# 959AI994/Multi-Gate-VAE

Measured on AMD Instinct MI355X. Metric: circuit-graphs/sec (train step), AIG-64k batch=64 per GPU, higher is better.
Workload: dtype f32 storage; dense products as bf16x3 split-precision MFMA, fp32 accumulate; 1 GPU; cfg2: DG_AE --type aig, 64 x 65536-node synthetic levelised DAGs per GPU (N=4194304, E=6558720, 120 levels), H=64, 4+4 rounds, layernorm, weights [1,4,4], negatives sampled; step includes the 7-scalar metrics copy (pinned, read one step behind); global_batch=64, parallelism=dp1

## Files before the change

include/mgvae_hip.h:

```cpp
#ifndef MGVAE_HIP_H
#define MGVAE_HIP_H
#include <stdint.h>
#ifdef __cplusplus
extern "C" {
#endif

#ifndef MGV_OK
#define MGV_OK 0
#define MGV_EINVAL (-1)
#define MGV_EUNSUPPORTED (-2)
#endif

int mgv_abi_version(void);

int mgv_struct_stage_fwd(int H, int64_t N, const float* h_in, const int32_t* nbr_ptr, const int32_t* nbr_idx,
                         const uint8_t* xcls, const float* xtab, int C, const float* Wc, const float* bc,
                         const float* Whh, const float* bhh, const float* ln_w, const float* ln_b, float ln_eps,
                         float* h_out, void* stream);
int mgv_struct_stage_bwd(int H, int64_t N, const float* h_in, const int32_t* nbr_ptr, const int32_t* nbr_idx,
                         const uint8_t* xcls, const float* xtab, int C, const float* Wc, const float* WcT,
                         const float* bc, const float* Whh, const float* WhhT, const float* bhh,
                         const float* ln_w, const float* ln_b, float ln_eps, const float* gy_direct,
                         const float* gy_agg, float* g_direct_out, float* g_agg_out, float* dWc, float* dbc,
                         float* dWhh, float* dbhh, float* dxtab, float* dln_w, float* dln_b, void* stream);
// ... 264 lines not shown
                      int32_t* scratch, int64_t scratch_ints, void* stream);
int mgv_colour_rep_rows(int64_t C, const int32_t* rep, const int32_t* nbr_ptr, const int32_t* prev, const uint8_t* xcls, int heavy_row,
                        int32_t* rptr, int32_t* own, uint8_t* xrep, int32_t* n_heavy, int32_t* scratch, int64_t scratch_ints, void* stream);
int mgv_colour_rep_lists(int64_t C, const int32_t* rep, const int32_t* nbr_ptr, const int32_t* nbr_idx, const int32_t* prev, const int32_t* rptr,
                         int32_t* ent, int32_t* row, void* stream);
int mgv_sorted_key_counts(int64_t n, const int32_t* sorted_keys, int64_t K, int32_t* counts, void* stream);
int mgv_seg_level_work_ints(int64_t G);
int mgv_seg_level_scan(int64_t G, const int32_t* counts, int seg, int32_t* work, int64_t work_ints, void* stream);
int mgv_seg_level_fill(int64_t G, int64_t n_seg, const int32_t* gid, int seg, int base, const int32_t* work, int32_t* seg_ptr, int32_t* out_row,
                       int32_t* gid_next, int32_t* counts_next, void* stream);

int mgv_digcn_scales(int64_t N, const int32_t* list_ptr, const int32_t* opp_ptr, float alpha, float beta, int self_loops,
                     float* r, float* c, void* stream);
int mgv_digcn_gather(int H, int64_t N, const float* y, const int32_t* nbr_ptr, const int32_t* nbr_idx, const float* outer,
                     const float* inner, const float* mask, int self_loops, int relu, int heavy_n, const int32_t* heavy_nodes,
                     float* out, void* stream);
int mgv_digcn_class_fwd(int H, int64_t N, const uint8_t* xcls, const float* T, int C, const int32_t* nbr_ptr, const int32_t* nbr_idx,
                        const float* outer, const float* inner, int self_loops, int relu, float* out, void* stream);
int mgv_digcn_class_bwd_ws_floats(int H, int64_t N);
int mgv_digcn_class_bwd(int H, int64_t N, const uint8_t* xcls, int C, const int32_t* nbr_ptr, const int32_t* nbr_idx, const float* outer,
                        const float* inner, int self_loops, const float* z, const float* dz, float* dT, float* workspace,
                        int64_t workspace_floats, void* stream);

#ifdef __cplusplus
}
#endif
#endif
```

multi-gate-vae_amd/csrc/linear_x3.hip:

```cpp
#include "mgv_x3.h"
#include "mgv_slab.h"
#include "../../include/mgvae_hip.h"

namespace mgv {

struct LinX3Args {
    int64_t N;
    const float* X1; int K1; int ld1;
    const float* X2; int K2; int ld2;
    const __bf16* wpack;
    const float* b;
    float* Y; int ldy;
    const float* R; int ldr;
    float* Y2; int ldy2;
    const float* dY; int lddy;
    float* dW; float* db;
    float* slab;
    const int32_t* order; const int32_t* tile_start; const int32_t* tile_count; const int32_t* tile_slot; const int32_t* tile_list;
    int64_t g_ntiles; int64_t g_wstride;
};

template <int M>
struct LinSplit {
    static_assert(M % 16 == 0, "column tiles of 16");
// ... 301 lines not shown
        if (tid < G::F4G) s_part[tid] = dbs;
        __syncthreads();
        constexpr int QPR = M / 4;
        if (tid < M) {
            const int c4 = tid / 4, e = tid % 4;
            float sum = 0.f;
            for (int t = c4; t < G::F4G && t < G::NT; t += QPR) { const float4 v = s_part[t]; sum += e == 0 ? v.x : e == 1 ? v.y : e == 2 ? v.z : v.w; }
            slab[M * K + tid] = sum;
        }
    }
}

template <int M, int K, int NW, int WI, bool GROUPED = false>
__global__ __launch_bounds__(64 * NW) void k_linear_wgrad_x3(LinX3Args a) {
    linear_wgrad_x3_body<M, K, NW, WI, GROUPED, false, 0>(a);
}

template <int M, int K, int NW, int WI, int KSR>
__global__ __launch_bounds__(64 * NW) __attribute__((amdgpu_waves_per_eu(4))) void k_linear_bwd_x3(LinX3Args a) {
    linear_wgrad_x3_body<M, K, NW, WI, false, true, KSR>(a);
}

__global__ __launch_bounds__(256) void k_wpack_bf16x3(const float* W, int R, int K, int ldw, int transpose, __bf16* hi, __bf16* lo) {
    const int total = R * K, ksn = K / 32;
    for (int o = blockIdx.x * 256 + threadIdx.x; o < total; o += gridDim.x * 256) {
        const int blk = o >> 9, within = o & 511, lane = within >> 3, e = within & 7;
        const int rt = blk / ksn, ks = blk % ksn;
        const int row = rt * 16 + (lane & 15), k = ks * 32 + (lane >> 4) * 8 + e;
        const float v = transpose ? W[(int64_t)k * ldw + row] : W[(int64_t)row * ldw + k];
        __bf16 h, l;
        split_bf16(v, h, l);
        hi[o] = h; lo[o] = l;
    }
}

template <int M, int K, bool GROUPED = false>
int launch_linear_fwd_x3(const LinX3Args& a, hipStream_t st) {
    using G = LinFwdGeom<M, K>;
    static bool set = false;
    if (!set) { hipFuncSetAttribute(reinterpret_cast<const void*>(k_linear_fwd_x3<M, K, GROUPED>), hipFuncAttributeMaxDynamicSharedMemorySize, 160 * 1024); set = true; }
    const int64_t ntiles = a.order ? a.g_ntiles : (a.N + kTileRows - 1) / kTileRows;
    int per_cu = 160 * 1024 / G::smem_bytes;
    per_cu = per_cu > 4 ? 4 : per_cu;
    hipLaunchKernelGGL((k_linear_fwd_x3<M, K, GROUPED>), dim3(grid_for(ntiles, per_cu)), dim3(kThreads), G::smem_bytes, st, a);
    MGV_LAUNCH_RET();
}

template <int M, int K, int NW, int WI, bool GROUPED = false>
int launch_linear_wgrad_x3(const LinX3Args& a, int64_t ws_floats, hipStream_t st) {
    using G = LinWgGeom<M, K, NW, WI>;
    static bool set = false;
    if (!set) { hipFuncSetAttribute(reinterpret_cast<const void*>(k_linear_wgrad_x3<M, K, NW, WI, GROUPED>), hipFuncAttributeMaxDynamicSharedMemorySize, 160 * 1024); set = true; }
    const int64_t ntiles = a.order ? a.g_ntiles : (a.N + kTileRows - 1) / kTileRows;
    int per_cu = 160 * 1024 / G::smem_bytes;
    const int cap = 1024 / G::NT;
    per_cu = per_cu > cap ? cap : per_cu;
// ... 149 lines not shown
```

multi-gate-vae_amd/csrc/mgv_x3.h:

```cpp
#pragma once
#include "mgv_common.h"

typedef __bf16 bf16x8 __attribute__((ext_vector_type(8)));
typedef __bf16 bf16x4 __attribute__((ext_vector_type(4)));

namespace mgv {

__device__ __forceinline__ void split_bf16(float x, __bf16& hi, __bf16& lo) {
    hi = (__bf16)x;
    lo = (__bf16)(x - (float)hi);
}

__device__ __forceinline__ void split4(const float4& v, bf16x4& hi, bf16x4& lo) {
    __bf16 h0, h1, h2, h3, l0, l1, l2, l3;
    split_bf16(v.x, h0, l0); split_bf16(v.y, h1, l1); split_bf16(v.z, h2, l2); split_bf16(v.w, h3, l3);
    hi = bf16x4{h0, h1, h2, h3};
    lo = bf16x4{l0, l1, l2, l3};
}

__device__ __forceinline__ bf16x8 ldfrag(const __bf16* p) { return *reinterpret_cast<const bf16x8*>(p); }
__device__ __forceinline__ bf16x8 ldfrag_global(const __bf16* p) {
    return *(const __attribute__((address_space(1))) bf16x8*)p;
}
__device__ __forceinline__ void st_bf4(__bf16* p, const bf16x4& v) { *reinterpret_cast<bf16x4*>(p) = v; }

__device__ __forceinline__ f32x4 mfma_bf16(const bf16x8& a, const bf16x8& b, f32x4 c) {
    return __builtin_amdgcn_mfma_f32_16x16x32_bf16(a, b, c, 0, 0, 0);
}

__device__ __forceinline__ void mma_x3(f32x4& c, const bf16x8& ahi, const bf16x8& alo, const bf16x8& bhi, const bf16x8& blo) {
    c = mfma_bf16(alo, bhi, c);
    c = mfma_bf16(ahi, blo, c);
    c = mfma_bf16(ahi, bhi, c);
}

typedef __bf16 bf16x4v __attribute__((ext_vector_type(4)));
__device__ __forceinline__ bf16x8 ldfrag_tr(const __bf16* plane, int ld, int k0, int c0) {
    const int lane = threadIdx.x & 63, q = lane >> 4, i16 = lane & 15;
    const __bf16* p = plane + (k0 + 8 * q + (i16 >> 2)) * ld + c0 + 4 * (i16 & 3);
    const bf16x4v lo = __builtin_amdgcn_ds_read_tr16_b64_v4bf16((__attribute__((address_space(3))) bf16x4v*)p);
// ... 20 lines not shown
```

multi-gate-vae_amd/deepgate/_hip.py:

```python
import ctypes
import os
import re

import torch

_HERE = os.path.dirname(os.path.abspath(__file__))
_PKG_ROOT = os.path.dirname(_HERE)
_REPO_ROOT = os.path.dirname(_PKG_ROOT)
LIB_PATH = os.environ.get('MGV_LIB', os.path.join(_PKG_ROOT, 'csrc', 'libmgvae_hip.so'))
HEADER_PATH = os.path.join(_REPO_ROOT, 'include', 'mgvae_hip.h')

_CTYPE = (('int64_t', ctypes.c_int64), ('uint64_t', ctypes.c_uint64), ('int32_t', ctypes.c_int32),
          ('float', ctypes.c_float), ('double', ctypes.c_double), ('int', ctypes.c_int))


class HipLibraryError(RuntimeError):
    pass


def parse_header(path=HEADER_PATH):
    with open(path) as f:
        text = f.read()
    text = re.sub(r'/\*.*?\*/', '', text, flags=re.S)
    text = re.sub(r'//[^\n]*', '', text)
# ... 19 lines not shown

_lib = None
_sigs = None


def load():
    global _lib, _sigs
    if _lib is not None:
        return _lib
    if not os.path.exists(LIB_PATH):
        raise HipLibraryError('%s not found: build it with `make -C %s` (or __graft_entry__.build()); '
                              'there is no CPU fallback for the DG_AE hot path' % (LIB_PATH, os.path.dirname(LIB_PATH)))
    lib = ctypes.CDLL(LIB_PATH)
    sigs = parse_header()
    for name, types in sigs.items():
        try:
            fn = getattr(lib, name)
        except AttributeError:
            raise HipLibraryError('%s is declared in %s but not exported by %s' % (name, HEADER_PATH, LIB_PATH))
        fn.argtypes = types
        fn.restype = ctypes.c_int
    _lib, _sigs = lib, sigs
    return lib


class _TensorPtr(ctypes.c_void_p):
    _keep = None


def ptr(t):
    if t is None:
        return None
    p = _TensorPtr(t.data_ptr())
    p._keep = t
    return p


_raw_stream = getattr(torch._C, '_cuda_getCurrentRawStream', None)


def stream():
    if _raw_stream is not None:
        return ctypes.c_void_p(_raw_stream(torch.cuda.current_device()))
    return ctypes.c_void_p(torch.cuda.current_stream().cuda_stream)


# ... 52 lines not shown
```

multi-gate-vae_amd/deepgate/_model_base.py:

```python
import os

import torch
from torch import nn

from . import ops
from .arch.mlp import MLP
from .arch.tfmlp import TFMlpAggr
from .data import plan_of
from .digae_layer import DirectedInnerProductDecoder
from .sampling import NegativeEdges, negative_sampling, negative_sampling_device

EPS = 1e-15
DEVICE_SAMPLER = True
MAX_LOGSTD = 10


class FunctionalModel(nn.Module):
    ENCODER_ATTR = 'struct_encoder'
    GATES = ()

    def __init__(self, struct_encoder, num_rounds=1, dim_hidden=128, enable_encode=True, enable_reverse=True):
        super().__init__()
        setattr(self, self.ENCODER_ATTR, struct_encoder)
        self.decoder = DirectedInnerProductDecoder()
        self.hs_linear = nn.Linear(dim_hidden * 2, dim_hidden)
        self.hs_decompose = nn.Linear(dim_hidden, dim_hidden * 2)
        self.num_rounds = num_rounds
        self.enable_encode = enable_encode
        self.enable_reverse = enable_reverse
        self.dim_hidden = dim_hidden
        self.dim_mlp = 32
        for name, _ in self.GATES:
            setattr(self, 'aggr_%s_func' % name, TFMlpAggr(dim_hidden * 2, dim_hidden))
        for name, _ in self.GATES:
            setattr(self, 'update_%s_func' % name, nn.GRU(dim_hidden, dim_hidden))
        self.readout_prob = MLP(dim_hidden, self.dim_mlp, 1, num_layer=3, p_drop=0.2, norm_layer='batchnorm',
                                act_layer='relu')
        self.last_confusion = None
        self.last_link_metrics = None

    def _sweep_params(self):
        parts = [getattr(self, 'aggr_%s_func' % n).composed(getattr(self, 'update_%s_func' % n)) for n, _ in self.GATES]
        return [torch.stack([p[i] for p in parts]) for i in range(5)]

    def forward(self, G, after_hs=None):
        if self.num_rounds < 1:
            raise ValueError('num_rounds must be >= 1')
        plan = plan_of(G, [gid for _, gid in self.GATES])
        dev = self.hs_linear.weight.device
        rows = torch.eye(6, dtype=torch.float32, device=dev)
        enc = getattr(self, self.ENCODER_ATTR)
        s, t = enc(None, None, G.edge_index, plan=plan, classes=(rows, plan.xcls))
        hs = ops.linear(s, self.hs_linear.weight, self.hs_linear.bias, x2=t)
        self._hs_ready = torch.cuda.Event()
        self._hs_ready.record()
        self._hs_pass = None
        self.after_hs_out = after_hs(hs) if after_hs is not None else None
        hs_in = self._hs_pass if self._hs_pass is not None else hs
        self._hs_pass = None
        hf = ops.FuncSweepFn.apply(plan, hs_in, *self._sweep_params())
        for _ in range(self.num_rounds - 1):
            au, Wvc, bvc, bih, _ = self._sweep_params()
            hf = ops.FuncSweepFn.apply(plan, hs_in, au, Wvc, bvc, bih, None, hf, self._round_gh(plan, hf))
        return hs, hf
# ... 131 lines not shown
```

multi-gate-vae_amd/deepgate/digae_layer.py:

```python
import torch
import torch.nn as nn

from . import ops
from .arch.gcn_conv import AggConv
from .graph_plan import GraphPlan

MAX_FEATURE_CLASSES = 8


def feature_classes(x):
    rows, inv = torch.unique(x, dim=0, return_inverse=True)
    if rows.shape[0] > MAX_FEATURE_CLASSES:
        return None
    return rows.to(torch.float32), inv.to(torch.uint8).contiguous()


class DirectedInnerProductDecoder(nn.Module):

    def forward(self, s, t, edge_index, sigmoid=True):
        return ops.edge_dot(s, t, edge_index, sigmoid)

    def forward_all(self, s, t, sigmoid=True):
        return ops.pair_scores(s, t, sigmoid)

# ... 147 lines not shown
        for aggr, gru in ((self.aggr, self.update), (self.aggr_r, self.update_r)):
            w_ih = gru.weight_ih_l0
            w_m = w_ih[:, :H]
            w_x = torch.nn.functional.pad(w_ih[:, H:], (0, pad))
            xrow = torch.cat([ops.linear(xp, w_x[g * H:(g + 1) * H], gru.bias_ih_l0[g * H:(g + 1) * H]) for g in range(3)], dim=1)
            args += [xrow, w_m @ aggr.msg.weight, w_m @ aggr.msg.bias, gru.weight_hh_l0, gru.bias_hh_l0]
        ln_w = self.ln.weight if self.layernorm else None
        ln_b = self.ln.bias if self.layernorm else None
        return ops.StructEncoderRowsFn.apply(plan, self.num_rounds, *args, ln_w, ln_b)

    def forward(self, x, edge_index, plan=None, classes=None):
        if classes is None:
            if x.shape[1] != self.dim_feature:
                raise ValueError('expected %d node features, got %d' % (self.dim_feature, x.shape[1]))
            classes = feature_classes(x)
        if classes is None:
            return self._forward_rows(x, edge_index, plan)
        rows, xcls = classes
        if rows.shape[1] != self.dim_feature:
            raise ValueError('expected %d node features, got %d' % (self.dim_feature, rows.shape[1]))
        if plan is None:
            plan = GraphPlan(edge_index, xcls.shape[0])
        rows = rows.to(self.update.weight_ih_l0.device)
        f = self._composed(self.aggr, self.update, rows)
        r = self._composed(self.aggr_r, self.update_r, rows)
        ln_w = self.ln.weight if self.layernorm else None
        ln_b = self.ln.bias if self.layernorm else None
        return ops.StructEncoderFn.apply(plan, xcls, self.num_rounds, *f, *r, ln_w, ln_b)


class DirectMultiGCNEncoder(nn.Module):
    def __init__(self, dim_feature=3, dim_hidden=128, s_rounds=1, t_rounds=1, enable_reverse=True, layernorm=False):
        super().__init__()
        self.source_conv = MultiGCNEncoder(s_rounds, dim_hidden, dim_feature, enable_reverse, layernorm)
        self.target_conv = MultiGCNEncoder(t_rounds, dim_hidden, dim_feature, enable_reverse, layernorm)

    def forward(self, s, t, edge_index, plan=None, classes=None):
        if plan is None:
            plan = GraphPlan(edge_index, s.shape[0])
        cs = classes if classes is not None else feature_classes(s)
        ct = cs if (classes is not None or t is s) else feature_classes(t)
        return self.source_conv(s, edge_index, plan, cs), self.target_conv(t, edge_index, plan, ct)
```

multi-gate-vae_amd/deepgate/ops.py:

```python
from collections import namedtuple

import torch

from . import _hip
from ._hip import HipLibraryError, check, ptr

import os

F32 = torch.float32
I32 = torch.int32
U8 = torch.uint8
LN_EPS = 1e-5

PRECISION = os.environ.get('MGV_PRECISION', 'x3')
FIRST_STAGE_TABLE = True


def use_x3(H):
    return PRECISION == 'x3' and H in (32, 64)


def split_bf16(w):
    hi = w.to(torch.bfloat16)
    lo = (w - hi.to(torch.float32)).to(torch.bfloat16)
    return hi, lo


def frag_order(w):
    R, K = w.shape
    return w.reshape(R // 16, 16, K // 32, 4, 8).permute(0, 2, 3, 1, 4).reshape(-1)


def _pack_into(out, off, W, transpose):
    R, K = (W.shape[1], W.shape[0]) if transpose else W.shape
    n = W.numel()
    if W.dtype != F32 or not W.is_cuda or W.stride(1) != 1:
        raise HipLibraryError('weight must be an fp32 GPU matrix with contiguous rows')
    base = out.data_ptr() + 2 * off
    _hip.call('mgv_wpack_bf16x3', ptr(W), R, K, W.stride(0), int(transpose), _hip.ctypes.c_void_p(base),
              _hip.ctypes.c_void_p(base + 2 * n))
    return off + 2 * n


def stage_wpack(Wc, Whh):
    out = torch.empty(4 * (Wc.numel() + Whh.numel()), dtype=torch.bfloat16, device=Wc.device)
    off = 0
    for w, tr in ((Wc, False), (Whh, False), (Wc, True), (Whh, True)):
        off = _pack_into(out, off, w, tr)
    return out


def sweep_wpack(Wvc):
    out = torch.empty(4 * Wvc.numel(), dtype=torch.bfloat16, device=Wvc.device)
    off = 0
    for g in range(Wvc.shape[0]):
        off = _pack_into(out, off, Wvc[g], False)
        off = _pack_into(out, off, Wvc[g], True)
    return out


def linear_wpack(W):
    out = torch.empty(2 * W.numel(), dtype=torch.bfloat16, device=W.device)
    _pack_into(out, 0, W, False)
    return out


def _zeros_like_params(*ts):
    return [torch.zeros_like(t) for t in ts]


def _heavy_args(heavy, H, device):
    if heavy is None or heavy[0] == 0:
        return 0, None, None
    n, nodes = heavy
    return n, ptr(nodes), ptr(workspace(2 * n * H, device, tag='heavy'))


def struct_stage_fwd(h_in, nbr_ptr, nbr_idx, xcls, xtab, Wc, bc, Whh, bhh, ln_w, ln_b, out=None, wpack=None, heavy=None, table_own=None, n_rows=None,
                     stats_out=None, tagged=True):
    N, H = h_in.shape
    if n_rows is not None:
        N = int(n_rows)
    if table_own is not None:
        N = table_own.numel()
    check(h_in, F32, 'h_in'); check(nbr_ptr, I32, 'nbr_ptr'); check(nbr_idx, I32, 'nbr_idx'); check(xcls, U8, 'xcls')
    for n, t in (('xtab', xtab), ('Wc', Wc), ('bc', bc), ('Whh', Whh), ('bhh', bhh)):
        check(t, F32, n)
    check(ln_w, F32, 'ln_w'); check(ln_b, F32, 'ln_b')
    assert nbr_ptr.numel() == N + 1 and xcls.numel() == N
    assert Wc.shape == (3 * H, H) and Whh.shape == (3 * H, H) and xtab.shape[1] == 3 * H
    h_out = (torch.empty(N, H, dtype=F32, device=h_in.device) if out is None else out)
# ... 97 lines not shown
                     dict(idx=st['idx'], n_rows=st['C'], src='stacked', own=st['own']))
            out.append(HalfRound(rev, st['C'], st['ptr'], xcls=st['xcls'], heavy=st['heavy'], expand=st['cid'] if k + 1 == q else None,
                                 grad=grad, gsrc=gsrc, **lists))
        elif k == 0 and first is not None:
            cid, C, tp, ti, tx = first
            out.append(HalfRound(rev, C, tp, ti, tx, None, src='ones', expand=None if table_mode else cid, grad='pairs', gsrc=(cid, p, i)))
        elif k == 1 and table_mode:
            out.append(HalfRound(rev, N, p, plan.tagged_idx(rev, first[0]), xcls, plan.heavy(rev), table_own=first[0]))
        else:
            out.append(HalfRound(rev, N, p, i, xcls, plan.heavy(rev), src='ones' if k == 0 else 'prev'))
    return out


class StructEncoderFn(torch.autograd.Function):

    @staticmethod
    def forward(ctx, plan, xcls, rounds, xtab_f, Wc_f, bc_f, Whh_f, bhh_f, xtab_r, Wc_r, bc_r, Whh_r, bhh_r, ln_w, ln_b):
        N = plan.N
        H = Whh_f.shape[1]
        dev = Whh_f.device
        par = [t.detach().contiguous() for t in (xtab_f, Wc_f, bc_f, Whh_f, bhh_f, xtab_r, Wc_r, bc_r, Whh_r, bhh_r)]
        lw = ln_w.detach().contiguous() if ln_w is not None else None
        lb = ln_b.detach().contiguous() if ln_b is not None else None
        packs = (stage_wpack(par[1], par[3]), stage_wpack(par[6], par[8])) if use_x3(H) else (None, None)
        quot = plan.quotient(xcls, 2 * rounds) if (QUOTIENT and FIRST_STAGE_TABLE and rounds > 0 and N > 0 and Whh_f.is_cuda) else []
        first = plan.first_stage_classes(xcls) if (not quot and FIRST_STAGE_TABLE and rounds > 0 and N > 0) else None
        sched = half_round_schedule(plan, xcls, rounds, H, use_x3(H), first, quot)
        keep_stats = lw is not None and use_x3(H) and H == 64
        states, stats = [], []
        h = torch.ones(1, H, dtype=F32, device=dev) if quot else None
        for r in sched:
            if r.src == 'ones':
                h = torch.ones(r.rows, H, dtype=F32, device=dev)
            elif r.src == 'stacked':
                h = torch.cat([h.index_select(0, r.own), h])
            states.append(None if r.grad == 'pairs' else h)
            stats.append(torch.empty(r.rows, 2, dtype=F32, device=dev) if keep_stats else None)
            h = struct_stage_fwd(h, r.ptr, r.idx, r.xcls, *(par[5:] if r.rev else par[:5]), lw, lb, wpack=packs[int(r.rev)], heavy=r.heavy,
                                 table_own=r.table_own, n_rows=r.n_rows, stats_out=stats[-1], tagged=r.tagged)
            if r.expand is not None:
                table, h = h, torch.empty(N, H, dtype=F32, device=dev)
                _hip.call('mgv_class_expand', H, N, ptr(table), ptr(r.expand), ptr(h))
        if not sched:
            h = torch.ones(N, H, dtype=F32, device=dev)
        ctx.plan, ctx.packs, ctx.sched = plan, packs, sched
        ctx.par, ctx.lw, ctx.lb, ctx.states, ctx.stats = par, lw, lb, states, stats
        return h

    @staticmethod
    def backward(ctx, gy):
        plan, par, lw, lb = ctx.plan, ctx.par, ctx.lw, ctx.lb
        H, dev = gy.shape[1], gy.device
        dlw = torch.zeros_like(lw) if lw is not None else None
        dlb = torch.zeros_like(lb) if lb is not None else None
        acc = [dict(zip(('dxtab', 'dWc', 'dbc', 'dWhh', 'dbhh', 'dln_w', 'dln_b'), _zeros_like_params(*w) + [dlw, dlb])) for w in (par[:5], par[5:])]
        g_direct, g_agg = gy.contiguous(), None
        for k in range(len(ctx.sched) - 1, -1, -1):
            r, h_in = ctx.sched[k], ctx.states[k]
            if r.grad == 'pairs':
                cid, p, i = r.gsrc
                gsum = torch.zeros(r.rows, H, dtype=F32, device=dev)
                ws = workspace(_hip.call_value('mgv_class_pull_sum_ws_floats', H, plan.N, r.rows), dev)
                _hip.call('mgv_class_pull_sum', H, plan.N, ptr(g_direct), ptr(g_agg), ptr(p), ptr(i), ptr(cid), r.rows, ptr(gsum), ptr(ws), ws.numel())
                g_direct, g_agg, h_in = gsum, None, torch.ones(r.rows, H, dtype=F32, device=dev)
            elif r.grad == 'sum_levels':
                (order, levels), p, i = r.gsrc
                g_direct, g_agg = _seg_sums(H, levels, order, g_direct, g_agg, p, i), None
            elif r.grad == 'above':
                own_levels, own_rows, ent_levels, ent_rows = r.gsrc
                g_direct, g_agg = _seg_sums(H, own_levels, own_rows, g_direct) + _seg_sums(H, ent_levels, ent_rows, g_agg), None
            g_direct, g_agg = struct_stage_bwd(h_in, r.ptr, r.idx, r.xcls, *(par[5:] if r.rev else par[:5]), lw, lb, g_direct, g_agg, acc[int(r.rev)],
                                               need_input_grad=(k > 0), wpack=ctx.packs[int(r.rev)], heavy=r.heavy, table_own=r.table_own,
                                               n_rows=r.n_rows, stats=ctx.stats[k], tagged=r.tagged)
        ctx.states = ctx.stats = None
        f, r = acc
        return (None, None, None, f['dxtab'], f['dWc'], f['dbc'], f['dWhh'], f['dbhh'],
                r['dxtab'], r['dWc'], r['dbc'], r['dWhh'], r['dbhh'], dlw, dlb)

# ... 28 lines not shown
        acc = {}
        for tag, w in (('f', par[:5]), ('r', par[5:])):
            acc[tag] = [torch.zeros_like(t) for t in w]
            acc[tag] += [w[1].t().contiguous(), w[3].t().contiguous()]
        dlw = torch.zeros_like(lw) if lw is not None else None
        dlb = torch.zeros_like(lb) if lb is not None else None
        g_direct, g_agg = gy.contiguous(), None
        k = len(ctx.states) - 1
        for _ in range(ctx.rounds):
            for rev in (True, False):
                p, i = plan.csr(rev)
                w = par[5:] if rev else par[:5]
                g = acc['r' if rev else 'f']
                gd = torch.empty(N, H, dtype=F32, device=dev) if k > 0 else None
                ga = torch.empty(N, H, dtype=F32, device=dev) if k > 0 else None
                _hip.call('mgv_struct_stage_rows_bwd', H, N, ptr(ctx.states[k]), ptr(p), ptr(i), ptr(w[0]), ptr(w[1]), ptr(g[5]), ptr(w[2]),
                          ptr(w[3]), ptr(g[6]), ptr(w[4]), ptr(lw), ptr(lb), LN_EPS, ptr(g_direct), ptr(g_agg), ptr(gd), ptr(ga),
                          ptr(g[1]), ptr(g[2]), ptr(g[3]), ptr(g[4]), ptr(g[0]), ptr(dlw), ptr(dlb))
                g_direct, g_agg = gd, ga
                k -= 1
        ctx.states = None
        f, r = acc['f'], acc['r']
        return (None, None, f[0], f[1], f[2], f[3], f[4], r[0], r[1], r[2], r[3], r[4], dlw, dlb)


_LIN_X3 = {}


def _lin_x3(M, K):
    if PRECISION != 'x3':
        return False
    key = (int(M), int(K))
    if key not in _LIN_X3:
        _LIN_X3[key] = bool(_hip.call_value('mgv_linear_x3_supported', *key))
    return _LIN_X3[key]


FUSED_LINEAR_BWD = os.environ.get('MGV_FUSED_LINEAR_BWD', '1') != '0'


def _lin_bwd_x3(M, K):
    if PRECISION != 'x3':
        return False
    key = ('bwd', int(M), int(K))
    if key not in _LIN_X3:
        _LIN_X3[key] = bool(_hip.call_value('mgv_linear_bwd_x3_supported', int(M), int(K)))
# ... 359 lines not shown
            _hip.call('mgv_func_sweep_fwd', H, N, T, plan.num_levels, ltp, ptr(plan.order), ptr(plan.tile_start),
                      ptr(plan.tile_count), ptr(plan.tile_slot), ptr(plan.in_ptr), ptr(plan.in_src), ptr(hsd), ptr(hf),
                      *[ptr(t) for t in par], ptr(ghd), ptr(hp))
        ctx.plan, ctx.par, ctx.ltp, ctx.wpack = plan, par, ltp, wpack
        ctx.save_for_backward(hsd, hf, hp, ghd)
        return hf

    @staticmethod
    def backward(ctx, ghf):
        global _SWEEP_BWD_EVENT
        plan, par = ctx.plan, ctx.par
        hs, hf, hp, ghd = ctx.saved_tensors
        if hp is None and ghf.is_cuda:
            _SWEEP_BWD_EVENT = torch.cuda.Event()
            _SWEEP_BWD_EVENT.record()
        N, H = hs.shape
        T = par[0].shape[0]
        dev = hs.device
        ghf = check(ghf.contiguous(), F32, 'ghf')
        ghs = (torch.empty if ctx.wpack is not None else torch.zeros)(N, H, dtype=F32, device=dev)
        dzb = torch.empty(N, 2 * H, dtype=F32, device=dev)
        alpha = torch.empty(max(plan.E, 1), dtype=F32, device=dev)
        dsc = torch.empty(max(plan.E, 1), dtype=F32, device=dev)
        grads = [torch.zeros_like(t) for t in par]
        d_gh = g_hprev = None
        if hp is not None:
            d_gh = torch.zeros(N, 3 * H, dtype=F32, device=dev)
            g_hprev = torch.zeros(N, H, dtype=F32, device=dev)
        rnd = (ptr(ghd), ptr(hp), ptr(d_gh), ptr(g_hprev))
        if ctx.wpack is not None:
            scratch, stp, hv, ha = _sweep_bwd_prep(plan, T, H, dev)
            _hip.call('mgv_func_sweep_bwd_x3', H, N, T, plan.num_levels, ctx.ltp, ptr(plan.order), *_sweep_rows(plan),
                      plan.n_active, ptr(plan.tile_start), ptr(plan.tile_count), ptr(plan.tile_slot), ptr(plan.slot_tiles), stp,
                      ptr(plan.in_ptr), ptr(plan.in_src), ptr(plan.out_ptr), ptr(plan.out_dst), ptr(plan.out_slot),
                      ptr(plan.gslot), ptr(hs), ptr(hf), ptr(par[0]), ptr(ctx.wpack), ptr(par[2]), ptr(par[3]), ptr(par[4]),
                      ptr(ghf), ptr(ghs), ptr(dzb), ptr(alpha), ptr(dsc), *[ptr(g) for g in grads], ptr(scratch),
                      scratch.numel(), plan.HEAVY_ROW if hv is not None else 0, *ha, *rnd)
            if hv is not None:
                pw = workspace(hv['S'] * H, dev)
                _hip.call('mgv_sweep_pull_heavy', H, hv['K'], ptr(hv['nodes']), ptr(hv['node_seg_ptr']), hv['S'], ptr(hv['seg_e0']), ptr(hv['seg_e1']),
                          ptr(plan.out_dst), ptr(plan.out_slot), ptr(plan.gslot), ptr(alpha), ptr(dsc), ptr(dzb), ptr(par[0]), ptr(pw), ptr(ghs))
        else:
            WvcT = par[1].transpose(1, 2).contiguous()
            _hip.call('mgv_func_sweep_bwd', H, N, T, plan.num_levels, ctx.ltp, ptr(plan.order), ptr(plan.tile_start),
                      ptr(plan.tile_count), ptr(plan.tile_slot), ptr(plan.in_ptr), ptr(plan.in_src), ptr(plan.out_ptr),
                      ptr(plan.out_dst), ptr(plan.out_slot), ptr(plan.gslot), ptr(hs), ptr(hf), ptr(par[0]), ptr(par[1]),
                      ptr(WvcT), ptr(par[2]), ptr(par[3]), ptr(par[4]), ptr(ghf), ptr(ghs), ptr(dzb), ptr(alpha), ptr(dsc),
# ... 881 lines not shown
```

Before: 1012 graphs/s.

## Batch weight-space composition, bf16x3 packing and grad zeroing into grouped launches

Adds a batched small-GEMM kernel and a batched bf16x3 weight-pack kernel, each driven by a job table passed as a kernel argument. Per-gate weight composition, its backward, the weight packing and the zeroing of parameter gradients now run as a few grouped launches instead of many small torch ops and kernel launches. The aim is to cut kernel-launch and Python dispatch overhead on the tiny weight-space operations in each train step. In exchange it adds host-side overlap checks on every call and custom autograd functions whose correctness rests on hand-computed strides and pointer offsets.

Result: no change. 1021 graphs/s, median of 6 (+0.9%).

```diff
diff --git a/include/mgvae_hip.h b/include/mgvae_hip.h
--- a/include/mgvae_hip.h
+++ b/include/mgvae_hip.h
@@ -310,6 +310,29 @@
                         const float* inner, int self_loops, const float* z, const float* dz, float* dT, float* workspace,
                         int64_t workspace_floats, void* stream);
 
+typedef struct mgv_gemm_job {
+    const float* A;
+    const float* B;
+    float* C;
+    const float* col_bias;
+    const float* row_bias;
+    const float* u;
+    const float* v;
+    int32_t a_rs, a_cs, b_rs, b_cs, c_rs, c_cs;
+    int32_t M, N, K, accumulate;
+} mgv_gemm_job;
+#define MGV_GEMM_JOBS_PER_LAUNCH 32
+int mgv_small_gemm_batch(int n_jobs, const mgv_gemm_job* jobs, void* stream);
+
+typedef struct mgv_wpack_job {
+    const float* W;
+    void* hi;
+    void* lo;
+    int32_t R, K, ldw, transpose;
+} mgv_wpack_job;
+#define MGV_WPACK_JOBS_PER_LAUNCH 64
+int mgv_wpack_bf16x3_batch(int n_jobs, const mgv_wpack_job* jobs, void* stream);
+
 #ifdef __cplusplus
 }
 #endif
diff --git a/multi-gate-vae_amd/csrc/linear_x3.hip b/multi-gate-vae_amd/csrc/linear_x3.hip
--- a/multi-gate-vae_amd/csrc/linear_x3.hip
+++ b/multi-gate-vae_amd/csrc/linear_x3.hip
@@ -347,16 +347,7 @@
 }
 
 __global__ __launch_bounds__(256) void k_wpack_bf16x3(const float* W, int R, int K, int ldw, int transpose, __bf16* hi, __bf16* lo) {
-    const int total = R * K, ksn = K / 32;
-    for (int o = blockIdx.x * 256 + threadIdx.x; o < total; o += gridDim.x * 256) {
-        const int blk = o >> 9, within = o & 511, lane = within >> 3, e = within & 7;
-        const int rt = blk / ksn, ks = blk % ksn;
-        const int row = rt * 16 + (lane & 15), k = ks * 32 + (lane >> 4) * 8 + e;
-        const float v = transpose ? W[(int64_t)k * ldw + row] : W[(int64_t)row * ldw + k];
-        __bf16 h, l;
-        split_bf16(v, h, l);
-        hi[o] = h; lo[o] = l;
-    }
+    wpack_planes(W, R, K, ldw, transpose, hi, lo, blockIdx.x * 256 + threadIdx.x, gridDim.x * 256);
 }
 
 template <int M, int K, bool GROUPED = false>
diff --git a/multi-gate-vae_amd/csrc/mgv_x3.h b/multi-gate-vae_amd/csrc/mgv_x3.h
--- a/multi-gate-vae_amd/csrc/mgv_x3.h
+++ b/multi-gate-vae_amd/csrc/mgv_x3.h
@@ -16,6 +16,19 @@
     split_bf16(v.x, h0, l0); split_bf16(v.y, h1, l1); split_bf16(v.z, h2, l2); split_bf16(v.w, h3, l3);
     hi = bf16x4{h0, h1, h2, h3};
     lo = bf16x4{l0, l1, l2, l3};
+}
+
+__device__ __forceinline__ void wpack_planes(const float* W, int R, int K, int ldw, int transpose, __bf16* hi, __bf16* lo, int first, int step) {
+    const int total = R * K, ksn = K / 32;
+    for (int o = first; o < total; o += step) {
+        const int blk = o >> 9, within = o & 511, lane = within >> 3, e = within & 7;
+        const int rt = blk / ksn, ks = blk % ksn;
+        const int row = rt * 16 + (lane & 15), k = ks * 32 + (lane >> 4) * 8 + e;
+        const float v = transpose ? W[(int64_t)k * ldw + row] : W[(int64_t)row * ldw + k];
+        __bf16 h, l;
+        split_bf16(v, h, l);
+        hi[o] = h; lo[o] = l;
+    }
 }
 
 __device__ __forceinline__ bf16x8 ldfrag(const __bf16* p) { return *reinterpret_cast<const bf16x8*>(p); }
diff --git a/multi-gate-vae_amd/csrc/weight_space.hip b/multi-gate-vae_amd/csrc/weight_space.hip
--- /dev/null
+++ b/multi-gate-vae_amd/csrc/weight_space.hip
@@ -0,0 +1,209 @@
+#include <stdint.h>
+
+#include "mgv_x3.h"
+#include "mgvae_hip.h"
+
+namespace mgv {
+
+constexpr int kGemmTile = 16;
+constexpr int kGemmKT = 32;
+
+struct GemmTable {
+    mgv_gemm_job job[MGV_GEMM_JOBS_PER_LAUNCH];
+    int32_t block0[MGV_GEMM_JOBS_PER_LAUNCH + 1];
+    int32_t n;
+};
+static_assert(sizeof(GemmTable) <= 4096, "the job table must fit the kernel arguments");
+
+struct WpackTable {
+    mgv_wpack_job job[MGV_WPACK_JOBS_PER_LAUNCH];
+    int32_t block0[MGV_WPACK_JOBS_PER_LAUNCH + 1];
+    int32_t n;
+};
+static_assert(sizeof(WpackTable) <= 4096, "the job table must fit the kernel arguments");
+
+template <class Table>
+__device__ __forceinline__ int job_of_block(const Table& t, int b) {
+    int j = 0;
+    while (j + 1 < t.n && b >= t.block0[j + 1]) ++j;
+    return j;
+}
+
+__global__ __launch_bounds__(256) void k_small_gemm_batch(const GemmTable t) {
+    __shared__ float sA[kGemmTile][kGemmKT + 1];
+    __shared__ float sB[kGemmKT][kGemmTile + 1];
+    const int j = job_of_block(t, blockIdx.x);
+    const mgv_gemm_job& J = t.job[j];
+    const int M = J.M, N = J.N, K = J.K;
+    const int64_t a_rs = J.a_rs, a_cs = J.a_cs, b_rs = J.b_rs, b_cs = J.b_cs;
+    const float* __restrict__ A = J.A;
+    const float* __restrict__ B = J.B;
+    const int b = blockIdx.x - t.block0[j], tiles_n = (N + kGemmTile - 1) / kGemmTile;
+    const int m0 = (b / tiles_n) * kGemmTile, n0 = (b % tiles_n) * kGemmTile;
+    const int tid = threadIdx.x, tx = tid & 15, ty = tid >> 4;
+    const bool a_k_minor = a_cs == 1 || a_rs != 1, b_n_minor = b_cs == 1 || b_rs != 1;
+    float acc = 0.f;
+    for (int k0 = 0; k0 < K; k0 += kGemmKT) {
+        for (int e = tid; e < kGemmTile * kGemmKT; e += 256) {
+            const int am = a_k_minor ? e / kGemmKT : e % kGemmTile, ak = a_k_minor ? e % kGemmKT : e / kGemmTile;
+            sA[am][ak] = (m0 + am < M && k0 + ak < K) ? A[(m0 + am) * a_rs + (k0 + ak) * a_cs] : 0.f;
+            const int bk = b_n_minor ? e / kGemmTile : e % kGemmKT, bn = b_n_minor ? e % kGemmTile : e / kGemmKT;
+            sB[bk][bn] = (k0 + bk < K && n0 + bn < N) ? B[(k0 + bk) * b_rs + (n0 + bn) * b_cs] : 0.f;
+        }
+        __syncthreads();
+        const int kn = K - k0 < kGemmKT ? K - k0 : kGemmKT;
+        if (kn == kGemmKT) {
+#pragma unroll
+            for (int kk = 0; kk < kGemmKT; ++kk) acc = fmaf(sA[ty][kk], sB[kk][tx], acc);
+        } else {
+            for (int kk = 0; kk < kn; ++kk) acc = fmaf(sA[ty][kk], sB[kk][tx], acc);
+        }
+        __syncthreads();
+    }
+    const int m = m0 + ty, n = n0 + tx;
+    if (m < M && n < N) {
+        float r = acc;
+        if (J.col_bias) r += J.col_bias[m];
+        if (J.row_bias) r += J.row_bias[n];
+        if (J.u) r = fmaf(J.u[m], J.v[n], r);
+        float* c = J.C + ((int64_t)m * J.c_rs + (int64_t)n * J.c_cs);
+        if (J.accumulate) r += *c;
+        *c = r;
+    }
+}
+
+__global__ __launch_bounds__(256) void k_wpack_bf16x3_batch(const WpackTable t) {
+    const int j = job_of_block(t, blockIdx.x);
+    const mgv_wpack_job& J = t.job[j];
+    const int nb = t.block0[j + 1] - t.block0[j];
+    wpack_planes(J.W, J.R, J.K, J.ldw, J.transpose, static_cast<__bf16*>(J.hi), static_cast<__bf16*>(J.lo),
+                 (blockIdx.x - t.block0[j]) * 256 + threadIdx.x, nb * 256);
+}
+
+struct Region {
+    uintptr_t p;
+    int64_t rows, cols, rs, cs;
+    uintptr_t lo() const { return p; }
+    uintptr_t hi() const { return p + 4 * (uintptr_t)((rows - 1) * rs + (cols - 1) * cs + 1); }
+};
+
+static bool region_ok(const Region& r) {
+    return r.rs >= 0 && r.cs >= 0 && (r.rows - 1) * r.rs + (r.cols - 1) * r.cs < INT32_MAX;
+}
+
+static bool region_injective(const Region& r) {
+    if ((r.rows > 1 && r.rs == 0) || (r.cols > 1 && r.cs == 0)) return false;
+    if (r.rows == 1 || r.cols == 1) return true;
+    return r.rs > (r.cols - 1) * r.cs || r.cs > (r.rows - 1) * r.rs;
+}
+
+static bool region_lines(const Region& r, int64_t& w, int64_t& ld) {
+    if (r.rows == 1 && (r.cs == 1 || r.cols == 1)) { w = r.cols; ld = 0; return true; }
+    if (r.cols == 1 && r.rs == 1) { w = r.rows; ld = 0; return true; }
+    if (r.cs == 1 || r.cols == 1) { w = r.cols; ld = r.rs; return ld > 0; }
+    if (r.rs == 1) { w = r.rows; ld = r.cs; return ld > 0; }
+    return false;
+}
+
+static bool regions_disjoint(const Region& x, const Region& y) {
+    if (x.hi() <= y.lo() || y.hi() <= x.lo()) return true;
+    int64_t wx, ldx, wy, ldy;
+    if (!region_lines(x, wx, ldx) || !region_lines(y, wy, ldy)) return false;
+    const int64_t ld = ldx ? ldx : ldy;
+    if (ld == 0 || (ldy && ldy != ld) || wx > ld || wy > ld) return false;
+    const int64_t diff = (int64_t)y.p - (int64_t)x.p;
+    if (diff % 4 != 0) return false;
+    const int64_t d = (((diff / 4) % ld) + ld) % ld;
+    return d >= wx && d + wy <= ld;
+}
+
+static int gemm_regions(const mgv_gemm_job& j, Region& out, Region* in ) {
+    out = Region{(uintptr_t)j.C, j.M, j.N, j.c_rs, j.c_cs};
+    int n = 0;
+    if (j.K > 0) {
+        in[n++] = Region{(uintptr_t)j.A, j.M, j.K, j.a_rs, j.a_cs};
+        in[n++] = Region{(uintptr_t)j.B, j.K, j.N, j.b_rs, j.b_cs};
+    }
+    if (j.col_bias) in[n++] = Region{(uintptr_t)j.col_bias, 1, j.M, 0, 1};
+    if (j.row_bias) in[n++] = Region{(uintptr_t)j.row_bias, 1, j.N, 0, 1};
+    if (j.u) in[n++] = Region{(uintptr_t)j.u, 1, j.M, 0, 1};
+    if (j.v) in[n++] = Region{(uintptr_t)j.v, 1, j.N, 0, 1};
+    return n;
+}
+
+}
+
+extern "C" int mgv_small_gemm_batch(int n_jobs, const mgv_gemm_job* jobs, void* stream) {
+    using namespace mgv;
+    MGV_CHECK_ARG(n_jobs >= 0 && (n_jobs == 0 || jobs));
+    for (int i = 0; i < n_jobs; ++i) {
+        const mgv_gemm_job& j = jobs[i];
+        MGV_CHECK_ARG(j.C && j.M >= 1 && j.N >= 1 && j.K >= 0 && (j.K == 0 || (j.A && j.B)) && (j.u == nullptr) == (j.v == nullptr));
+        MGV_CHECK_ARG(j.a_rs >= 0 && j.a_cs >= 0 && j.b_rs >= 0 && j.b_cs >= 0);
+        Region out, in[6];
+        const int n_in = gemm_regions(j, out, in);
+        MGV_CHECK_ARG(region_ok(out) && region_injective(out));
+        for (int a = 0; a < n_in; ++a) MGV_CHECK_ARG(region_ok(in[a]));
+    }
+    for (int i = 0; i < n_jobs; ++i) {
+        Region oi, ii[6], oj, ij[6];
+        gemm_regions(jobs[i], oi, ii);
+        for (int k = 0; k < n_jobs; ++k) {
+            const int n_in = gemm_regions(jobs[k], oj, ij);
+            if (k > i) MGV_CHECK_ARG(regions_disjoint(oi, oj));
+            for (int a = 0; a < n_in; ++a) MGV_CHECK_ARG(regions_disjoint(oi, ij[a]));
+        }
+    }
+    hipStream_t st = static_cast<hipStream_t>(stream);
+    for (int first = 0; first < n_jobs; first += MGV_GEMM_JOBS_PER_LAUNCH) {
+        GemmTable t;
+        t.n = n_jobs - first < MGV_GEMM_JOBS_PER_LAUNCH ? n_jobs - first : MGV_GEMM_JOBS_PER_LAUNCH;
+        int64_t blocks = 0;
+        for (int i = 0; i < t.n; ++i) {
+            t.job[i] = jobs[first + i];
+            t.block0[i] = (int32_t)blocks;
+            blocks += (int64_t)((t.job[i].M + kGemmTile - 1) / kGemmTile) * ((t.job[i].N + kGemmTile - 1) / kGemmTile);
+            MGV_CHECK_ARG(blocks < INT32_MAX);
+        }
+        for (int i = t.n; i <= MGV_GEMM_JOBS_PER_LAUNCH; ++i) t.block0[i] = (int32_t)blocks;
+        for (int i = t.n; i < MGV_GEMM_JOBS_PER_LAUNCH; ++i) t.job[i] = mgv_gemm_job{};
+        hipLaunchKernelGGL(k_small_gemm_batch, dim3((unsigned)blocks), dim3(256), 0, st, t);
+        const hipError_t e = hipGetLastError();
+        if (e != hipSuccess) return (int)e;
+    }
+    return MGV_OK;
+}
+
+extern "C" int mgv_wpack_bf16x3_batch(int n_jobs, const mgv_wpack_job* jobs, void* stream) {
+    using namespace mgv;
+    MGV_CHECK_ARG(n_jobs >= 0 && (n_jobs == 0 || jobs));
+    for (int i = 0; i < n_jobs; ++i) {
+        const mgv_wpack_job& j = jobs[i];
+        MGV_CHECK_ARG(j.W && j.hi && j.lo && j.R > 0 && j.K > 0 && j.R % 16 == 0 && j.K % 32 == 0 && j.ldw >= (j.transpose ? j.R : j.K));
+        MGV_CHECK_ARG((int64_t)j.R * j.K < INT32_MAX);
+    }
+    for (int i = 0; i < 2 * n_jobs; ++i)
+        for (int k = i + 1; k < 2 * n_jobs; ++k) {
+            const mgv_wpack_job &a = jobs[i / 2], &b = jobs[k / 2];
+            const uintptr_t pa = (uintptr_t)(i % 2 ? a.lo : a.hi), pb = (uintptr_t)(k % 2 ? b.lo : b.hi);
+            MGV_CHECK_ARG(pa + 2 * (uintptr_t)a.R * a.K <= pb || pb + 2 * (uintptr_t)b.R * b.K <= pa);
+        }
+    hipStream_t st = static_cast<hipStream_t>(stream);
+    for (int first = 0; first < n_jobs; first += MGV_WPACK_JOBS_PER_LAUNCH) {
+        WpackTable t;
+        t.n = n_jobs - first < MGV_WPACK_JOBS_PER_LAUNCH ? n_jobs - first : MGV_WPACK_JOBS_PER_LAUNCH;
+        int blocks = 0;
+        for (int i = 0; i < t.n; ++i) {
+            t.job[i] = jobs[first + i];
+            t.block0[i] = blocks;
+            const int nb = (t.job[i].R * t.job[i].K + 255) / 256;
+            blocks += nb > 1024 ? 1024 : nb;
+        }
+        for (int i = t.n; i <= MGV_WPACK_JOBS_PER_LAUNCH; ++i) t.block0[i] = blocks;
+        for (int i = t.n; i < MGV_WPACK_JOBS_PER_LAUNCH; ++i) t.job[i] = mgv_wpack_job{};
+        hipLaunchKernelGGL(k_wpack_bf16x3_batch, dim3((unsigned)blocks), dim3(256), 0, st, t);
+        const hipError_t e = hipGetLastError();
+        if (e != hipSuccess) return (int)e;
+    }
+    return MGV_OK;
+}
diff --git a/multi-gate-vae_amd/deepgate/_hip.py b/multi-gate-vae_amd/deepgate/_hip.py
--- a/multi-gate-vae_amd/deepgate/_hip.py
+++ b/multi-gate-vae_amd/deepgate/_hip.py
@@ -65,6 +65,10 @@
         fn.restype = ctypes.c_int
     _lib, _sigs = lib, sigs
     return lib
+
+
+def available():
+    return _lib is not None or os.path.exists(LIB_PATH)
 
 
 class _TensorPtr(ctypes.c_void_p):
diff --git a/multi-gate-vae_amd/deepgate/_model_base.py b/multi-gate-vae_amd/deepgate/_model_base.py
--- a/multi-gate-vae_amd/deepgate/_model_base.py
+++ b/multi-gate-vae_amd/deepgate/_model_base.py
@@ -40,6 +40,12 @@
         self.last_link_metrics = None
 
     def _sweep_params(self):
+        if ops.native_compose(self.hs_linear.weight):
+            raw = []
+            for n, _ in self.GATES:
+                a, g = getattr(self, 'aggr_%s_func' % n), getattr(self, 'update_%s_func' % n)
+                raw += [a.attn_lin.weight, a.msg_k.weight, g.weight_ih_l0, a.msg_v.weight, a.msg_v.bias, g.bias_ih_l0, g.bias_hh_l0]
+            return list(ops.SweepComposeFn.apply(*raw))
         parts = [getattr(self, 'aggr_%s_func' % n).composed(getattr(self, 'update_%s_func' % n)) for n, _ in self.GATES]
         return [torch.stack([p[i] for p in parts]) for i in range(5)]
 
diff --git a/multi-gate-vae_amd/deepgate/digae_layer.py b/multi-gate-vae_amd/deepgate/digae_layer.py
--- a/multi-gate-vae_amd/deepgate/digae_layer.py
+++ b/multi-gate-vae_amd/deepgate/digae_layer.py
@@ -193,8 +193,15 @@
         if plan is None:
             plan = GraphPlan(edge_index, xcls.shape[0])
         rows = rows.to(self.update.weight_ih_l0.device)
-        f = self._composed(self.aggr, self.update, rows)
-        r = self._composed(self.aggr_r, self.update_r, rows)
+        if ops.native_compose(rows, self.update.weight_ih_l0) and not rows.requires_grad:
+            raw = [t for a, g in ((self.aggr, self.update), (self.aggr_r, self.update_r))
+                   for t in (g.weight_ih_l0, g.bias_ih_l0, a.msg.weight, a.msg.bias)]
+            c = ops.StructComposeFn.apply(rows, *raw)
+            f = (*c[:3], self.update.weight_hh_l0, self.update.bias_hh_l0)
+            r = (*c[3:], self.update_r.weight_hh_l0, self.update_r.bias_hh_l0)
+        else:
+            f = self._composed(self.aggr, self.update, rows)
+            r = self._composed(self.aggr_r, self.update_r, rows)
         ln_w = self.ln.weight if self.layernorm else None
         ln_b = self.ln.bias if self.layernorm else None
         return ops.StructEncoderFn.apply(plan, xcls, self.num_rounds, *f, *r, ln_w, ln_b)
diff --git a/multi-gate-vae_amd/deepgate/ops.py b/multi-gate-vae_amd/deepgate/ops.py
--- a/multi-gate-vae_amd/deepgate/ops.py
+++ b/multi-gate-vae_amd/deepgate/ops.py
@@ -42,20 +42,85 @@
     return off + 2 * n
 
 
+NATIVE_COMPOSE = os.environ.get('MGV_NATIVE_COMPOSE', '1') != '0'
+
+
+def native_compose(*ts):
+    return NATIVE_COMPOSE and all(t.is_cuda and t.dtype == F32 for t in ts) and _hip.available()
+
+
+class _GemmJob(_hip.ctypes.Structure):
+    _fields_ = ([(n, _hip.ctypes.c_void_p) for n in ('A', 'B', 'C', 'col_bias', 'row_bias', 'u', 'v')] +
+                [(n, _hip.ctypes.c_int32) for n in ('a_rs', 'a_cs', 'b_rs', 'b_cs', 'c_rs', 'c_cs', 'M', 'N', 'K', 'accumulate')])
+
+
+class _WpackJob(_hip.ctypes.Structure):
+    _fields_ = ([(n, _hip.ctypes.c_void_p) for n in ('W', 'hi', 'lo')] +
+                [(n, _hip.ctypes.c_int32) for n in ('R', 'K', 'ldw', 'transpose')])
+
+
+def _vec(t):
+    return t if t is None or t.stride(0) == 1 or t.numel() <= 1 else t.contiguous()
+
+
+def gemm_job(C, A=None, B=None, col_bias=None, row_bias=None, u=None, v=None, accumulate=False):
+    M, N = C.shape
+    keep = [C, A, B, _vec(col_bias), _vec(row_bias), _vec(u), _vec(v)]
+    for t in keep:
+        if t is not None and (not t.is_cuda or t.dtype != F32):
+            raise HipLibraryError('weight-space operands must be fp32 GPU tensors')
+    K = 0 if A is None else A.shape[1]
+    assert (A is None) == (B is None) and (A is None or (A.shape[0] == M and B.shape == (K, N)))
+    assert all(t is None or t.numel() == n for t, n in zip(keep[3:], (M, N, M, N)))
+    j = _GemmJob(*[None if t is None else t.data_ptr() for t in (A, B, C, *keep[3:])],
+                 *(A.stride() if K else (0, 0)), *(B.stride() if K else (0, 0)), *C.stride(), M, N, K, int(bool(accumulate)))
+    return j, keep
+
+
+def _raw_job(C, c_rs, c_cs, M, N, K=0, A=None, a_rs=0, a_cs=0, B=None, b_rs=0, b_cs=0, col_bias=None, row_bias=None, u=None, v=None):
+    return _GemmJob(A, B, C, col_bias, row_bias, u, v, a_rs, a_cs, b_rs, b_cs, c_rs, c_cs, M, N, K, 0)
+
+
+def _dense(t, name='operand'):
+    return check(t if t.is_contiguous() else t.contiguous(), F32, name)
+
+
+def small_gemm_batch(jobs):
+    arr = (_GemmJob * len(jobs))(*[j[0] if isinstance(j, tuple) else j for j in jobs])
+    _hip.call('mgv_small_gemm_batch', len(jobs), arr)
+
+
+def _pack_all(out, mats):
+    off = 0
+    if not NATIVE_COMPOSE:
+        for W, tr in mats:
+            off = _pack_into(out, off, W, tr)
+        return
+    arr = (_WpackJob * len(mats))()
+    for j, (W, tr) in zip(arr, mats):
+        if W.dtype != F32 or not W.is_cuda or W.stride(1) != 1:
+            raise HipLibraryError('weight must be an fp32 GPU matrix with contiguous rows')
+        n, base = W.numel(), out.data_ptr() + 2 * off
+        j.W, j.hi, j.lo, j.ldw, j.transpose = W.data_ptr(), base, base + 2 * n, W.stride(0), int(tr)
+        j.R, j.K = (W.shape[1], W.shape[0]) if tr else W.shape
+        off += 2 * n
+    _hip.call('mgv_wpack_bf16x3_batch', len(mats), arr)
+
+
+def stage_wpacks(*pairs):
+    sizes = [4 * (Wc.numel() + Whh.numel()) for Wc, Whh in pairs]
+    out = torch.empty(sum(sizes), dtype=torch.bfloat16, device=pairs[0][0].device)
+    _pack_all(out, [(w, tr) for Wc, Whh in pairs for w, tr in ((Wc, False), (Whh, False), (Wc, True), (Whh, True))])
+    return out.split(sizes)
+
+
 def stage_wpack(Wc, Whh):
-    out = torch.empty(4 * (Wc.numel() + Whh.numel()), dtype=torch.bfloat16, device=Wc.device)
-    off = 0
-    for w, tr in ((Wc, False), (Whh, False), (Wc, True), (Whh, True)):
-        off = _pack_into(out, off, w, tr)
-    return out
+    return stage_wpacks((Wc, Whh))[0]
 
 
 def sweep_wpack(Wvc):
     out = torch.empty(4 * Wvc.numel(), dtype=torch.bfloat16, device=Wvc.device)
-    off = 0
-    for g in range(Wvc.shape[0]):
-        off = _pack_into(out, off, Wvc[g], False)
-        off = _pack_into(out, off, Wvc[g], True)
+    _pack_all(out, [(Wvc[g], tr) for g in range(Wvc.shape[0]) for tr in (False, True)])
     return out
 
 
@@ -66,7 +131,16 @@
 
 
 def _zeros_like_params(*ts):
-    return [torch.zeros_like(t) for t in ts]
+    real = [t for t in ts if t is not None]
+    if not real or not native_compose(*real):
+        return [None if t is None else torch.zeros_like(t) for t in ts]
+    sizes = [0 if t is None else (t.numel() + 63) // 64 * 64 for t in ts]
+    buf = torch.zeros(sum(sizes), dtype=F32, device=real[0].device)
+    out, off = [], 0
+    for t, s in zip(ts, sizes):
+        out.append(None if t is None else buf[off:off + t.numel()].view(t.shape))
+        off += s
+    return out
 
 
 def _heavy_args(heavy, H, device):
@@ -210,7 +284,7 @@
         par = [t.detach().contiguous() for t in (xtab_f, Wc_f, bc_f, Whh_f, bhh_f, xtab_r, Wc_r, bc_r, Whh_r, bhh_r)]
         lw = ln_w.detach().contiguous() if ln_w is not None else None
         lb = ln_b.detach().contiguous() if ln_b is not None else None
-        packs = (stage_wpack(par[1], par[3]), stage_wpack(par[6], par[8])) if use_x3(H) else (None, None)
+        packs = stage_wpacks((par[1], par[3]), (par[6], par[8])) if use_x3(H) else (None, None)
         quot = plan.quotient(xcls, 2 * rounds) if (QUOTIENT and FIRST_STAGE_TABLE and rounds > 0 and N > 0 and Whh_f.is_cuda) else []
         first = plan.first_stage_classes(xcls) if (not quot and FIRST_STAGE_TABLE and rounds > 0 and N > 0) else None
         sched = half_round_schedule(plan, xcls, rounds, H, use_x3(H), first, quot)
@@ -239,9 +313,9 @@
     def backward(ctx, gy):
         plan, par, lw, lb = ctx.plan, ctx.par, ctx.lw, ctx.lb
         H, dev = gy.shape[1], gy.device
-        dlw = torch.zeros_like(lw) if lw is not None else None
-        dlb = torch.zeros_like(lb) if lb is not None else None
-        acc = [dict(zip(('dxtab', 'dWc', 'dbc', 'dWhh', 'dbhh', 'dln_w', 'dln_b'), _zeros_like_params(*w) + [dlw, dlb])) for w in (par[:5], par[5:])]
+        zeros = _zeros_like_params(*par, lw, lb)
+        dlw, dlb = zeros[10:]
+        acc = [dict(zip(('dxtab', 'dWc', 'dbc', 'dWhh', 'dbhh', 'dln_w', 'dln_b'), z + [dlw, dlb])) for z in (zeros[:5], zeros[5:10])]
         g_direct, g_agg = gy.contiguous(), None
         for k in range(len(ctx.sched) - 1, -1, -1):
             r, h_in = ctx.sched[k], ctx.states[k]
@@ -316,6 +390,98 @@
         ctx.states = None
         f, r = acc['f'], acc['r']
         return (None, None, f[0], f[1], f[2], f[3], f[4], r[0], r[1], r[2], r[3], r[4], dlw, dlb)
+
+
+_ONE = {}
+
+
+def _ones_row(n, device):
+    one = _ONE.get(str(device))
+    if one is None:
+        one = _ONE[str(device)] = torch.ones(1, 1, dtype=F32, device=device)
+    return one.as_strided((1, n), (0, 0))
+
+
+class StructComposeFn(torch.autograd.Function):
+
+    @staticmethod
+    def forward(ctx, rows, *p):
+        rows, p = _dense(rows.detach(), 'rows'), [_dense(t.detach(), 'parameter') for t in p]
+        H = p[2].shape[0]
+        outs = []
+        for w_ih, b_ih, mw, mb in (p[:4], p[4:]):
+            w_m = w_ih[:, :H]
+            outs += [rows @ w_ih[:, H:].t() + b_ih, w_m @ mw, w_m @ mb]
+        ctx.save_for_backward(rows, *p)
+        return tuple(outs)
+
+    @staticmethod
+    @torch.autograd.function.once_differentiable
+    def backward(ctx, *g):
+        rows, *p = ctx.saved_tensors
+        H, (Cn, F_) = p[2].shape[0], rows.shape
+        W, H3 = H + F_, 3 * H
+        one, rp = _ones_row(1, rows.device).data_ptr(), rows.data_ptr()
+        g = [_dense(t, 'gradient') for t in g]
+        grads, jobs = [], []
+        for (w_ih, b_ih, mw, mb), (dxtab, dWc, dbc) in ((p[:4], g[:3]), (p[4:], g[3:])):
+            dw_ih, db_ih, dmw, dmb = (torch.empty_like(t) for t in (w_ih, b_ih, mw, mb))
+            wp, dxp, dWp, dbp, dwp = w_ih.data_ptr(), dxtab.data_ptr(), dWc.data_ptr(), dbc.data_ptr(), dw_ih.data_ptr()
+            jobs += [_raw_job(dwp, W, 1, H3, H, H, dWp, H, 1, mw.data_ptr(), 1, H, u=dbp, v=mb.data_ptr()),
+                     _raw_job(dwp + 4 * H, W, 1, H3, F_, Cn, dxp, 1, H3, rp, F_, 1),
+                     _raw_job(db_ih.data_ptr(), H3, 1, 1, H3, Cn, one, 0, 0, dxp, H3, 1),
+                     _raw_job(dmw.data_ptr(), H, 1, H, H, H3, wp, 1, W, dWp, H, 1),
+                     _raw_job(dmb.data_ptr(), 1, 1, H, 1, H3, wp, 1, W, dbp, 1, 1)]
+            grads += [dw_ih, db_ih, dmw, dmb]
+        small_gemm_batch(jobs)
+        return (None, *grads)
+
+
+class SweepComposeFn(torch.autograd.Function):
+    PER_SLOT = 7
+
+    @staticmethod
+    def forward(ctx, *p):
+        p = [_dense(t.detach(), 'parameter') for t in p]
+        T = len(p) // SweepComposeFn.PER_SLOT
+        H3, I, dev = p[2].shape[0], p[3].shape[1], p[0].device
+        au = torch.empty(T, I, dtype=F32, device=dev)
+        Wvc = torch.empty(T, H3, I, dtype=F32, device=dev)
+        bvc, bih, bhh = (torch.empty(T, H3, dtype=F32, device=dev) for _ in range(3))
+        jobs = []
+        for t in range(T):
+            aw, mk, w_ih, mv, mvb, b_ih, b_hh = p[7 * t:7 * t + 7]
+            torch.mm(aw[:, mk.shape[0]:], mk, out=au[t].unsqueeze(0))
+            torch.matmul(w_ih, mv, out=Wvc[t])
+            torch.matmul(w_ih, mvb, out=bvc[t])
+            jobs += [_raw_job(bih.data_ptr() + 4 * t * H3, H3, 1, 1, H3, row_bias=b_ih.data_ptr()),
+                     _raw_job(bhh.data_ptr() + 4 * t * H3, H3, 1, 1, H3, row_bias=b_hh.data_ptr())]
+        small_gemm_batch(jobs)
+        ctx.save_for_backward(*p)
+        return au, Wvc, bvc, bih, bhh
+
+    @staticmethod
+    @torch.autograd.function.once_differentiable
+    def backward(ctx, g_au, g_Wvc, g_bvc, g_bih, g_bhh):
+        p = ctx.saved_tensors
+        g_au, g_Wvc, g_bvc = (_dense(t, 'gradient') for t in (g_au, g_Wvc, g_bvc))
+        grads, jobs = [], []
+        for t in range(len(p) // SweepComposeFn.PER_SLOT):
+            aw, mk, w_ih, mv, mvb, b_ih, b_hh = p[7 * t:7 * t + 7]
+            out, I = mk.shape
+            H3, Hh = w_ih.shape
+            d_aw, d_mk, d_wih, d_mv, d_mvb = (torch.empty_like(x) for x in (aw, mk, w_ih, mv, mvb))
+            gau, gW, gb = g_au.data_ptr() + 4 * t * I, g_Wvc.data_ptr() + 4 * t * H3 * I, g_bvc.data_ptr() + 4 * t * H3
+            ap, wp = aw.data_ptr(), w_ih.data_ptr()
+            jobs += [_raw_job(d_aw.data_ptr(), 2 * out, 1, 1, out),
+                     _raw_job(d_aw.data_ptr() + 4 * out, 1, 1, out, 1, I, mk.data_ptr(), I, 1, gau, 1, 1),
+                     _raw_job(d_mk.data_ptr(), I, 1, out, I, u=ap + 4 * out, v=gau),
+                     _raw_job(d_wih.data_ptr(), Hh, 1, H3, Hh, I, gW, I, 1, mv.data_ptr(), 1, I, u=gb, v=mvb.data_ptr()),
+                     _raw_job(d_mv.data_ptr(), I, 1, Hh, I, H3, wp, 1, Hh, gW, I, 1),
+                     _raw_job(d_mvb.data_ptr(), 1, 1, Hh, 1, H3, wp, 1, Hh, gb, 1, 1)]
+            grads += [d_aw, d_mk, d_wih, d_mv, d_mvb, g_bih[t], g_bhh[t]]
+        small_gemm_batch(jobs)
+        return tuple(grads)
 
 
 _LIN_X3 = {}
@@ -721,7 +887,7 @@
         dzb = torch.empty(N, 2 * H, dtype=F32, device=dev)
         alpha = torch.empty(max(plan.E, 1), dtype=F32, device=dev)
         dsc = torch.empty(max(plan.E, 1), dtype=F32, device=dev)
-        grads = [torch.zeros_like(t) for t in par]
+        grads = _zeros_like_params(*par)
         d_gh = g_hprev = None
         if hp is not None:
             d_gh = torch.zeros(N, 3 * H, dtype=F32, device=dev)
```
